# Danderson123/Amira

Measured on AMD Instinct MI355X. Metric: gene-mers/s to corrected GeneMerGraph, higher is better.
Workload: dtype int32; 1 GPU; synthetic 1M reads x 60 genes, k=5, 20k-gene vocab: build + error-correction sweep (build, filter(3,1), correct, build, clip(5), correct, build); reads_per_gpu=1000000, genes_per_read=60, k=5, vocab=20000, gene_mers_per_gpu=56000000, final_nodes=472478, final_edges=1054844, multi_gpu=n/a

## Files before the change

amira_amd/csrc/amg_correct.h:

```cpp
#pragma once
#include "amg_device.h"

enum { RC_SKIP = 0, RC_COPY = 1, RC_DROP = 2, RC_TRIM = 3, RC_GAPPED = 4, RC_KEEP_ORIG = 5 };

struct CorrArgs {
  const int* tokens;
  const long long* read_off;
  const int* tok_node;
  const signed char* tok_dir;
  const unsigned char* read_fix;
  const long long* p0s;
  const long long* p0e;
  const long long* p1s;
  const long long* p1e;
  long long n0;
  const long long* pos_off;
  const long long* read_len;
  long long n_reads;
  int k, flip, have_pos;
  unsigned int* gflag;
  unsigned long long* max_bound;
  unsigned long long* lmask;
  unsigned long long* n_runs;
  unsigned char* cls;
  unsigned char* cls_final;
  int* r_start;
  int* r_end;
  unsigned int* bound;
  const long long* tmp_off;
  unsigned int* new_len;
  int* tmp_tok;
};

__device__ __forceinline__ void pos_base(const CorrArgs& a, long long off, const long long*& gs, const long long*& ge) {
  if (off < a.n0) {
    gs = a.p0s + off;
    ge = a.p0e + off;
  } else {
    gs = a.p1s + (off - a.n0);
    ge = a.p1e + (off - a.n0);
  }
}

__device__ __forceinline__ long long bcast_i64(long long v, int lane) {
  const unsigned int lo = (unsigned int)__builtin_amdgcn_readlane((int)(unsigned int)v, lane);
  const unsigned int hi = (unsigned int)__builtin_amdgcn_readlane((int)(unsigned int)((unsigned long long)v >> 32), lane);
  return (long long)(((unsigned long long)hi << 32) | lo);
}

__device__ __forceinline__ void wave_sync() {
  __builtin_amdgcn_fence(__ATOMIC_ACQ_REL, "wavefront");
  __builtin_amdgcn_wave_barrier();
}

struct __attribute__((aligned(16))) GapRec {
  int r, L0, start, end;
  long long t0, dst;
  unsigned long long mask;
  long long pad;
};

__device__ __forceinline__ unsigned long long gap_run_ends(unsigned long long lv, int start, int end) {
  const unsigned long long inside =
      (end >= 63 ? ~0ull : ((1ull << (end + 1)) - 1ull)) & ~((1ull << (start & 63)) - 1ull);
  return ~lv & inside & (lv >> 1);
}
__device__ __forceinline__ void gap_run_terminals(unsigned long long lv, int i, int& ps, int& pe) {
  ps = 63 - __clzll((long long)(lv & ((1ull << i) - 1ull)));
  pe = i + 1;
}

struct GapArgs {
  CorrArgs a;
  GView g;
  const GapRec* rec;
  const int* gapped_reads;
  long long n_gapped;
  int* pool;
  unsigned long long pool_cap;
  unsigned long long* pool_used;
  unsigned long long* status;
  int* cand;
  unsigned int cand_stride;
  unsigned char* final_cls;
  unsigned char* need_slow;
  const int* gq;
  const int4* qres;
  const int* qpool;
};

#define GF_MAXW 128
#define GF_MAXGAP 16
#define GF_POOL 384
#define GF_CAND 136
#define GF_MAXCOMBO 256
#define GM_INLINE 64
#define LEAN_CHUNK 32
#define CLS_READS 64
#define PACK_READS 64
enum {
  GS_NOT_TRIED = 1,
  GS_WINDOWS = 2,
  GS_RUNS = 3,
  GS_MEMO_UNFIT = 4,
  GS_RECORDS = 5,
  GS_COMBOS = 6,
  GS_CAND = 7,
  GS_CODES = 8
};
enum {
  GL_NO_SLOTS = 1,
  GL_ANSWERS = 2,
  GL_LONG = 3,
  GL_OTHER = 4,
  GL_CODES = 5
};

#define NWF_MAX_M 64
#define NWF_MAX_N 128
__device__ __forceinline__ bool nw_fast_ok(long long N, long long M) {
  return N <= NWF_MAX_N && M <= NWF_MAX_M && N > 0 && M > 0;
}

struct __attribute__((aligned(16))) NwRec {
  int r, M, N, pad;
  long long t0, dst;
  long long pdst;
  long long poff;
};

struct NwArgs {
  CorrArgs a;
  const NwRec* rec;
  long long* o_gs;
  long long* o_ge;
  const int* gapped_reads;
  long long n_gapped;
  const unsigned char* final_cls;
  const long long* big_off;
  unsigned char* big_buf;
  int allow_fast;
  int shortcuts;
  unsigned char* route;
};
enum { NW_ROUTE_NONE = 0, NW_ROUTE_EQUAL = 1, NW_ROUTE_CERT = 2, NW_ROUTE_FILL = 3, NW_ROUTE_LDS = 4, NW_ROUTE_GLOBAL = 5 };

struct PackArgs {
  CorrArgs a;
  const long long* new_idx;
  const long long* new_off;
  const unsigned char* final_cls;
  int* o_tok;
  long long* o_off;
  int* o_orig;
  unsigned char* o_changed;
  long long* o_src;
  const long long* pos_new;
  long long* o_posoff;
  long long* o_rl;
  long long out_reads, out_tokens;
  unsigned long long* dead_kept;
};

struct CorrSwitches {
  bool gap_memo;
  bool fast_gapped;
  bool lean_gapped;
  int fast_nw;
  int nw_shortcuts;
  const char* node_bound;
  bool routes;
  const char* gap_pool;
  const char* memo_spill;
};

struct CorrScratch {
  size_t per_read = 0;
  unsigned char *cls = nullptr, *final_cls = nullptr;
  int *r_start = nullptr, *r_end = nullptr;
  long long *nw_size = nullptr, *nw_off = nullptr;
  unsigned int *bound = nullptr, *new_len = nullptr, *flag = nullptr;
  long long *tmp_off = nullptr, *new_idx = nullptr, *new_off = nullptr;
  int* tmp_tok = nullptr;
  long long *plen = nullptr, *poffs = nullptr, *pos_new = nullptr;
  unsigned long long *max_bound = nullptr, *n_general = nullptr;
  unsigned long long* n_runs = nullptr;
  unsigned long long* dead_kept = nullptr;
  bool count_alive = false;
  DevBuf* glist = nullptr;
  DevBuf* cand = nullptr;
  DevBuf* pool = nullptr;
  DevBuf* need_slow = nullptr;
};

struct CorrCounts {
  long long tmp_total = 0, n_gapped = 0, total_runs = 0;
  unsigned long long max_bound = 0;
  bool carry = false;
  long long out_reads = 0, out_tokens = 0, big_total = 0, pos_total = 0;
  unsigned long long n_general = 0;
  long long n_queries = 0;
  int pool_retries = 0;
  bool lean_ran = false, fast_ran = false, memo = false;
};

static void fill_pos_args(amg_ctx* c, CorrArgs& a) {
  a.p0s = c->have_pos ? c->gene_start.as<long long>() : nullptr;
  a.p0e = c->have_pos ? c->gene_end.as<long long>() : nullptr;
  a.p1s = c->pos1_s.as<long long>();
  a.p1e = c->pos1_e.as<long long>();
  a.n0 = c->pos_n0;
  a.pos_off = (c->have_pos && !c->pos_identity) ? c->pos_off.as<long long>() : nullptr;
}

void corr_classify_launch(amg_ctx* c, const CorrArgs& a);
int corr_gapped(amg_ctx* c, const CorrSwitches& sw, const CorrScratch& S, const CorrArgs& a, CorrCounts& n);
int corr_nw_sizes(amg_ctx* c, const CorrSwitches& sw, const CorrScratch& S, const CorrArgs& a, long long n_gapped,
                  FetchList& shape);
int corr_grow_pos_pools(amg_ctx* c, const CorrCounts& n);
int corr_positions(amg_ctx* c, const CorrSwitches& sw, const CorrScratch& S, const CorrArgs& a, const CorrCounts& n,
                   unsigned char* route = nullptr);

int routes_begin(amg_ctx* c);
int routes_gapped(amg_ctx* c, const CorrScratch& S, const CorrCounts& n, const unsigned char* need_slow, const int* gq);
int routes_nw(amg_ctx* c, const CorrScratch& S, const CorrCounts& n);
int routes_end(amg_ctx* c, const CorrCounts& n);
```

amira_amd/csrc/amg_correct.hip:

```cpp
#include "amg_correct.h"

__global__ __launch_bounds__(256) void k_count_alive(const unsigned char* __restrict__ alive, long long n,
                                                     unsigned long long* out) {
  __shared__ unsigned int s_part[4];
  unsigned int c = 0;
  for (long long i = ((long long)blockIdx.x * blockDim.x + threadIdx.x) * 4; i < n; i += (long long)gridDim.x * blockDim.x * 4) {
    if (i + 4 <= n) {
      const unsigned int w = *reinterpret_cast<const unsigned int*>(alive + i);
      c += __popc(w & 0x01010101u);
    } else {
      for (long long j = i; j < n; ++j) c += alive[j] ? 1u : 0u;
    }
  }
  for (int d = 32; d > 0; d >>= 1) c += (unsigned int)__shfl_xor((int)c, d, 64);
  if ((threadIdx.x & 63) == 0) s_part[threadIdx.x >> 6] = c;
  __syncthreads();
  if (threadIdx.x == 0 && (s_part[0] | s_part[1] | s_part[2] | s_part[3]))
    atomicAdd(out, (unsigned long long)s_part[0] + s_part[1] + s_part[2] + s_part[3]);
}

__global__ __launch_bounds__(256) void k_corr_pack(PackArgs A) {
  const CorrArgs& a = A.a;
  const int lane = threadIdx.x & 63;
  const long long r = ((long long)blockIdx.x * 4 + (threadIdx.x >> 6)) * PACK_READS + lane;
  if (blockIdx.x == 0 && threadIdx.x == 0) A.o_off[A.out_reads] = A.out_tokens;
  long long dst = 0, src = 0;
  int n = 0;
  unsigned int dead = 0;
  if (r < a.n_reads && a.new_len[r] > 0) {
    dst = A.new_off[r];
    n = (int)a.new_len[r];
    const unsigned char fc = A.final_cls[r];
    if (fc == RC_KEEP_ORIG) {
      const long long nw = a.read_off[r + 1] - a.read_off[r] - a.k + 1;
      dead = nw <= 64 ? (unsigned int)(nw - __popcll(a.lmask[r])) : (unsigned int)nw;
    }
    long long poff = 0;
    if (fc == RC_GAPPED) {
      src = a.tmp_off[r] | (1ll << 62);
      if (a.have_pos) poff = A.pos_new[r];
    } else {
      const long long cut = fc == RC_TRIM ? a.r_start[r] : 0;
      src = a.read_off[r] + cut;
      if (a.have_pos) poff = (a.pos_off ? a.pos_off[r] : a.read_off[r]) + cut;
    }
    const long long q = A.new_idx[r];
    A.o_off[q] = dst;
    A.o_orig[q] = (int)r;
    A.o_changed[q] = (fc == RC_TRIM || fc == RC_GAPPED) ? 1 : 0;
    A.o_src[q] = fc == RC_GAPPED ? -1ll : src;
    if (a.have_pos) A.o_posoff[q] = poff;
    if (a.read_len) A.o_rl[q] = a.read_len[r];
  }
  if (__ballot(dead != 0u) != 0ull) {
    for (int d = 32; d > 0; d >>= 1) dead += (unsigned int)__shfl_xor((int)dead, d, 64);
    if (lane == 0) atomicAdd(A.dead_kept + 16 * (blockIdx.x & 15), (unsigned long long)dead);
  }
  if (__ballot(n > 0) == 0ull) return;
  for (int j0 = 0; j0 < PACK_READS; j0 += 4) {
    const int* sp[4];
    long long d[4];
    int nn[4], vt[4];
#pragma unroll
    for (int j = 0; j < 4; ++j) {
      nn[j] = __builtin_amdgcn_readlane(n, j0 + j);
      const long long sj = bcast_i64(src, j0 + j);
      d[j] = bcast_i64(dst, j0 + j);
      sp[j] = ((sj >> 62) & 1 ? a.tmp_tok : a.tokens) + (sj & ~(1ll << 62));
    }
#pragma unroll
    for (int j = 0; j < 4; ++j)
      if (lane < nn[j]) vt[j] = sp[j][lane];
#pragma unroll
    for (int j = 0; j < 4; ++j)
      if (lane < nn[j]) A.o_tok[d[j] + lane] = vt[j];
#pragma unroll
    for (int j = 0; j < 4; ++j)
      for (int i = 64 + lane; i < nn[j]; i += 64)
        A.o_tok[d[j] + i] = sp[j][i];
  }
}

static CorrSwitches read_switches() {
  auto is_one = [](const char* name) {
    const char* v = getenv(name);
    return v && v[0] == '1';
  };
  CorrSwitches sw;
  sw.gap_memo = !is_one("AMG_NO_GAP_MEMO");
  sw.fast_gapped = !is_one("AMG_NO_FAST_GAPPED");
  sw.lean_gapped = !is_one("AMG_NO_LEAN_GAPPED");
  sw.fast_nw = !is_one("AMG_NO_FAST_NW");
  sw.nw_shortcuts = !is_one("AMG_NW_NO_SHORTCUT");
  sw.node_bound = getenv("AMG_TEST_NODE_BOUND");
  sw.routes = is_one("AMG_CORR_ROUTES");
  sw.gap_pool = getenv("AMG_TEST_GAP_POOL");
  sw.memo_spill = getenv("AMG_TEST_MEMO_SPILL");
  return sw;
}

static int plan_per_read(amg_ctx* c, CorrScratch& S) {
  const size_t per_read = (size_t)(c->n_reads + 2);
  AMGCHK(c->s0.ensure(per_read * (1 + 1) + 64));
  AMGCHK(c->s1.ensure(per_read * sizeof(int) * 2 + per_read * sizeof(long long) * 2 + 64));
  AMGCHK(c->s2.ensure(per_read * sizeof(unsigned int) * 3));
  AMGCHK(c->s3.ensure(per_read * sizeof(long long) * 3));
  AMGCHK(c->gm_mask.ensure(per_read * sizeof(unsigned long long)));
  AMGCHK(c->gm_ctr.ensure((16 + 256 + 256 + 16) * sizeof(unsigned long long)));
  S.per_read = per_read;
  S.cls = c->s0.as<unsigned char>();
  S.final_cls = S.cls + per_read;
  S.r_start = c->s1.as<int>();
  S.r_end = S.r_start + per_read;
  S.nw_size = reinterpret_cast<long long*>(((uintptr_t)(S.r_end + per_read) + 15) & ~(uintptr_t)15);
  S.nw_off = S.nw_size + per_read;
  S.bound = c->s2.as<unsigned int>();
  S.new_len = S.bound + per_read;
  S.flag = S.new_len + per_read;
  S.tmp_off = c->s3.as<long long>();
  S.new_idx = S.tmp_off + per_read;
  S.new_off = S.new_idx + per_read;
  S.max_bound = S.n_general = c->status.as<unsigned long long>() + ST_MISC;
  S.n_runs = c->gm_ctr.as<unsigned long long>() + 16;
  S.dead_kept = S.n_runs + 256;
  S.count_alive = c->n_nodes >= (1ll << 20);
  S.glist = &c->c_orig;
  S.cand = &c->c_gstart;
  S.pool = &c->c_gend;
  S.need_slow = &c->c_changed;
  return AMG_OK;
}

static int plan_staging(amg_ctx* c, CorrScratch& S, long long tmp_total) {
  AMGCHK(c->c_tokens_buf.ensure((size_t)(tmp_total + 4) * sizeof(int)));
  AMGCHK(c->s4.ensure((size_t)(tmp_total + 4) * sizeof(int)));
  S.tmp_tok = c->s4.as<int>();
  return AMG_OK;
}

static int plan_positions(amg_ctx* c, CorrScratch& S, long long n_gapped) {
  AMGCHK(c->s5.ensure((size_t)(2 * (n_gapped + 2) + c->n_reads + 2) * sizeof(long long)));
  S.plen = c->s5.as<long long>();
  S.poffs = S.plen + (n_gapped + 2);
  S.pos_new = S.poffs + (n_gapped + 2);
  return AMG_OK;
}

static void corr_args(amg_ctx* c, const CorrScratch& S, CorrArgs& a) {
  a.tokens = c->tokens.as<int>();
  a.read_off = c->read_off.as<long long>();
  a.tok_node = c->tok_node.as<int>();
  a.tok_dir = c->tok_dir.as<signed char>();
  a.read_fix = c->read_fix.as<unsigned char>();
  fill_pos_args(c, a);
  a.read_len = c->have_read_len ? c->read_len.as<long long>() : nullptr;
  a.n_reads = c->n_reads;
  a.k = c->k;
  a.flip = c->two_v - 1;
  a.have_pos = c->have_pos ? 1 : 0;
  a.gflag = S.flag;
  a.max_bound = S.max_bound;
  a.lmask = c->gm_mask.as<unsigned long long>();
  a.n_runs = S.n_runs;
  a.cls = S.cls;
  a.cls_final = S.final_cls;
  a.r_start = S.r_start;
  a.r_end = S.r_end;
  a.bound = S.bound;
  a.tmp_off = S.tmp_off;
  a.new_len = S.new_len;
  a.tmp_tok = S.tmp_tok;
}

static int corr_classify(amg_ctx* c, const CorrScratch& S, const CorrArgs& a, CorrCounts& n) {
  hipStream_t st = c->stream;
  const long long R = c->n_reads;
  {
    ClearList cl;
    cl.add(S.bound, S.per_read * sizeof(unsigned int) * 3);
    cl.add(S.max_bound, sizeof(unsigned long long));
    cl.add(S.n_runs, (256 + 256 + 16) * sizeof(unsigned long long));
    AMGCHK(clear_many(c, cl));
  }
  if (R > 0) corr_classify_launch(c, a);
  if (S.count_alive)
    hipLaunchKernelGGL(k_count_alive, dim3(128), dim3(256), 0, st, c->node_alive.as<unsigned char>(), c->n_nodes,
                       S.dead_kept + 256);
  AMGCHK(prim_exscan_u32_pair(c, S.bound, S.tmp_off, S.flag, S.new_idx, (size_t)R));
  FetchList l;
  l.add(S.tmp_off + R);
  l.add(S.max_bound);
  l.add(S.new_idx + R);
  for (int i = 0; i < 16; ++i) l.add(S.n_runs + 16 * i);
  unsigned long long v[3 + 16];
  AMGCHK(fetch(c, l, v));
  n.tmp_total = (long long)v[0];
  n.max_bound = v[1];
  n.n_gapped = (long long)v[2];
  for (int i = 0; i < 16; ++i) n.total_runs += (long long)v[3 + i];
  n.carry = n.n_gapped > 0 && c->have_pos;
  return AMG_OK;
}

static int corr_shape(amg_ctx* c, const CorrSwitches& sw, CorrScratch& S, const CorrArgs& a, CorrCounts& n) {
  const long long R = c->n_reads;
  AMGCHK(prim_exscan_keep_and_len(c, S.new_len, S.new_idx, S.new_off, (size_t)R));
  FetchList shape;
  shape.add(S.new_idx + R);
  shape.add(S.new_off + R);
  if (n.carry) {
    AMGCHK(plan_positions(c, S, n.n_gapped));
    AMGCHK(corr_nw_sizes(c, sw, S, a, n.n_gapped, shape));
  }
  unsigned long long v[5] = {0, 0, 0, 0, 0};
  AMGCHK(fetch(c, shape, v));
  n.out_reads = (long long)v[0];
  n.out_tokens = (long long)v[1];
  n.big_total = (long long)v[2];
  n.pos_total = (long long)v[3];
  n.n_general = v[4];
  return AMG_OK;
}

static int ensure_outputs(amg_ctx* c, const CorrCounts& n) {
  AMGCHK(c->c_tokens_buf.ensure((size_t)(n.out_tokens + 64) * sizeof(int)));
  AMGCHK(c->c_read_off.ensure((size_t)(n.out_reads + 2) * sizeof(long long)));
  AMGCHK(c->c_orig.ensure((size_t)(n.out_reads + 2) * sizeof(int)));
  AMGCHK(c->c_changed.ensure((size_t)(n.out_reads + 2)));
  AMGCHK(c->c_src.ensure((size_t)(n.out_reads + 2) * sizeof(long long)));
  if (c->have_pos) AMGCHK(c->c_pos_off.ensure((size_t)(n.out_reads + 2) * sizeof(long long)));
  if (c->have_read_len) AMGCHK(c->c_read_len.ensure((size_t)(n.out_reads + 2) * sizeof(long long)));
  return AMG_OK;
}

static int corr_pack(amg_ctx* c, const CorrScratch& S, const CorrArgs& a, const CorrCounts& n) {
  PackArgs Pk;
  Pk.a = a;
  Pk.new_idx = S.new_idx;
  Pk.new_off = S.new_off;
  Pk.final_cls = S.final_cls;
  Pk.o_tok = c->c_tokens_buf.as<int>();
  Pk.o_off = c->c_read_off.as<long long>();
// ... 90 lines not shown
```

amira_amd/csrc/amg_correct_gapped.hip:

```cpp
#include "amg_correct.h"
#include "amg_wave_dfs.h"

__global__ __launch_bounds__(256) void k_corr_classify(CorrArgs a) {
  const long long rbase = ((long long)blockIdx.x * 4 + (threadIdx.x >> 6)) * CLS_READS;
  if (rbase >= a.n_reads) return;
  const int lane = threadIdx.x & 63;
  const long long r = rbase + lane;
  const bool have = r < a.n_reads;
  const long long t0 = have ? a.read_off[r] : 0;
  const long long n = have ? (a.read_off[r + 1] - t0) - a.k + 1 : 0;
  const bool look = have && n > 0 && a.read_fix[r] != 0;
  unsigned long long lv = 0;
  unsigned long long todo = __ballot(look && n <= 64);
  while (todo) {
    int who[4];
    long long tj[4];
    int nj[4], v[4];
#pragma unroll
    for (int q = 0; q < 4; ++q) {
      who[q] = todo ? __ffsll((long long)todo) - 1 : -1;
      if (todo) todo &= todo - 1ull;
      tj[q] = who[q] >= 0 ? bcast_i64(t0, who[q]) : 0;
      nj[q] = who[q] >= 0 ? __builtin_amdgcn_readlane((int)n, who[q]) : 0;
    }
#pragma unroll
    for (int q = 0; q < 4; ++q) v[q] = lane < nj[q] ? a.tok_node[tj[q] + lane] : -1;
#pragma unroll
    for (int q = 0; q < 4; ++q) {
      const unsigned long long m = __ballot(v[q] >= 0);
      if (lane == who[q]) lv = m;
    }
  }
  long long first = n, last = -1;
  unsigned int runs = 0, live = 0;
  if (look && n <= 64) {
    first = lv ? (long long)__ffsll((long long)lv) - 1 : n;
    last = lv ? 63 - (long long)__clzll((long long)lv) : -1;
    live = (unsigned int)__popcll(lv);
    const unsigned long long inside =
        lv ? ((last == 63 ? ~0ull : ((1ull << (last + 1)) - 1ull)) & ~((1ull << first) - 1ull)) : 0ull;
    runs = (unsigned int)__popcll(~lv & inside & (lv >> 1));
  }
  unsigned long long big = __ballot(look && n > 64);
  while (big) {
    const int w = __ffsll((long long)big) - 1;
    big &= big - 1ull;
    const long long tw = bcast_i64(t0, w), nw = bcast_i64(n, w);
    long long f = nw, l = -1;
    for (long long i = lane; i < nw; i += 64)
      if (a.tok_node[tw + i] >= 0) {
        f = f < i ? f : i;
        l = l > i ? l : i;
      }
    for (int d = 32; d > 0; d >>= 1) {
      const long long f2 = __shfl_xor(f, d, 64), l2 = __shfl_xor(l, d, 64);
      f = f < f2 ? f : f2;
      l = l > l2 ? l : l2;
    }
    unsigned int ru = 0, li = 0;
    if (l >= 0) {
      for (long long i = f + lane; i <= l; i += 64) {
        const bool none = a.tok_node[tw + i] < 0;
        li += none ? 0u : 1u;
        if (none && a.tok_node[tw + i + 1] >= 0) ++ru;
      }
      for (int d = 32; d > 0; d >>= 1) {
        ru += __shfl_xor(ru, d, 64);
        li += __shfl_xor(li, d, 64);
      }
    }
    if (lane == w) {
      first = f;
      last = l;
      runs = ru;
      live = li;
    }
  }
  const long long L = n + a.k - 1;
  unsigned char cls;
  int start = 0, end = -1;
  unsigned int bound = 0;
  unsigned int len_out = 0;
  if (n <= 0) {
    cls = RC_SKIP;
  } else if (!look) {
    cls = RC_COPY;
    len_out = (unsigned int)L;
  } else if (last < 0) {
    cls = RC_DROP;
  } else {
    start = (int)first;
    end = (int)last;
    if (runs == 0) {
      cls = RC_TRIM;
      len_out = (unsigned int)(end - start + a.k);
    } else {
      cls = RC_GAPPED;
      const unsigned int b1 = live + runs * (unsigned int)(2 * a.k) + (unsigned int)a.k;
      bound = b1 > (unsigned int)L ? b1 : (unsigned int)L;
    }
  }
  if (have) {
    a.cls[r] = cls;
    a.cls_final[r] = cls;
    a.r_start[r] = start;
    a.r_end[r] = end;
    a.bound[r] = bound;
    a.new_len[r] = len_out;
    a.gflag[r] = cls == RC_GAPPED ? 1u : 0u;
    a.lmask[r] = (cls == RC_GAPPED && n <= 64) ? lv : 0ull;
  }
  unsigned int mb = (have && cls == RC_GAPPED) ? bound : 0u;
  unsigned int nr = (have && cls == RC_GAPPED) ? runs : 0u;
  for (int d = 32; d > 0; d >>= 1) {
    const unsigned int o = (unsigned int)__shfl_xor((int)mb, d, 64);
    mb = mb > o ? mb : o;
    nr += (unsigned int)__shfl_xor((int)nr, d, 64);
  }
  if (lane == 0 && (unsigned long long)mb > *a.max_bound) atomicMax(a.max_bound, (unsigned long long)mb);
  if (lane == 0 && nr) atomicAdd(a.n_runs + 16 * (blockIdx.x & 15), (unsigned long long)nr);
}

void corr_classify_launch(amg_ctx* c, const CorrArgs& a) {
  hipLaunchKernelGGL(k_corr_classify, dim3(nblk(a.n_reads, 4 * CLS_READS)), dim3(256), 0, c->stream, a);
}

#define DFS_MAX (2 * AMG_MAX_K + 4)

struct PathSink {
  int* buf;
  long long used;
  int n_paths;
};

__device__ void dfs_paths(const GView& g, int s, int sdir, int e, int distance, PathSink* sink) {
  int node[DFS_MAX], dir[DFS_MAX];
  long long cur[DFS_MAX], lim[DFS_MAX];
  int depth = 0;
  node[0] = s;
  dir[0] = sdir;
  bool entering = true;
  while (depth >= 0) {
    if (entering) {
      int L = depth + 1;
      if (node[depth] == e && L <= distance) {
        if (sink->buf) {
          int* o = sink->buf + sink->used;
          o[0] = L;
          for (int j = 0; j < L; ++j) {
            o[1 + j] = node[j];
            o[1 + L + j] = dir[j];
          }
        }
        sink->used += 1 + 2 * L;
        sink->n_paths += 1;
        --depth;
        entering = false;
        continue;
      }
      if (L - 1 > distance) {
        --depth;
        entering = false;
        continue;
      }
      long long row = 2ll * node[depth] + (dir[depth] == 1 ? 0 : 1);
      const int4 rw = g.lrows[row];
      cur[depth] = rw.x;
      lim[depth] = rw.x + rw.y;
      entering = false;
    }
    bool pushed = false;
    while (cur[depth] < lim[depth]) {
      const int2 ent = g.lent[cur[depth]++];
      int t = ent.x;
      bool seen = false;
      for (int j = 0; j <= depth; ++j) seen = seen || (node[j] == t);
      if (seen) continue;
      node[depth + 1] = t;
      dir[depth + 1] = ent.y;
      ++depth;
      entering = true;
      pushed = true;
      break;
    }
    if (!pushed) --depth;
  }
}

__device__ __forceinline__ int oriented_tok(const GView& g, int n, int d, int j) {
  const int* nt = g.n_tok + (long long)n * g.k;
  return d == 1 ? nt[j] : g.flip - nt[g.k - 1 - j];
}

struct GapIter {
  long long t0;
  const int* tok_node;
  int start, end, i;
  int ps, pe;
  __device__ bool next() {
    while (i <= end) {
      int idx = i++;
      if (tok_node[t0 + idx] < 0) {
        if (tok_node[t0 + idx - 1] >= 0) ps = idx - 1;
        if (tok_node[t0 + idx + 1] >= 0) {
          pe = idx + 1;
          return true;
        }
      }
    }
    return false;
  }
};

__device__ __forceinline__ bool cand_better(int shared, unsigned long long csum, int n, int best_shared,
                                            unsigned long long best_sum, unsigned long long best_len) {
  return shared > best_shared || (shared == best_shared && csum * best_len > best_sum * (unsigned long long)n);
}

__device__ int build_candidate(const GapArgs& A, long long t0, int start, int end, const int* rec,
                               int n_gaps, unsigned long long combo, int* out_node, signed char* out_dir) {
  int n = 0;
  int q = 0;
  int i = start;
  int prev_pe = -1;
  while (i <= end) {
    if (q < n_gaps && rec[4 * q] == i) {
      int ps = rec[4 * q], pe = rec[4 * q + 1], np = rec[4 * q + 2];
      unsigned long long div = 1;
      for (int j = q + 1; j < n_gaps; ++j) div *= (unsigned long long)rec[4 * j + 2];
      int pick = (int)((combo / div) % (unsigned long long)np);
      const int* p = A.pool + rec[4 * q + 3];
      for (int s = 0; s < pick; ++s) p += 1 + 2 * p[0];
      int L = p[0];
      if (prev_pe == ps && n > 0) --n;
      for (int j = 0; j < L; ++j) {
        out_node[n] = p[1 + j];
        out_dir[n] = (signed char)p[1 + L + j];
        ++n;
      }
      prev_pe = pe;
      i = pe;
      ++q;
      if (!(q < n_gaps && rec[4 * q] == pe)) i = pe + 1;
    } else {
      out_node[n] = A.a.tok_node[t0 + i];
      out_dir[n] = A.a.tok_dir[t0 + i];
      ++n;
      ++i;
    }
  }
  return n;
}

__global__ __launch_bounds__(64) void k_corr_gapped(GapArgs A) {
  const CorrArgs& a = A.a;
  const GView& g = A.g;
  const long long gtid = (long long)blockIdx.x * blockDim.x + threadIdx.x;
  const long long gstride = (long long)gridDim.x * blockDim.x;
  int* my = A.cand + gtid * (long long)A.cand_stride;
  for (long long gi = gtid; gi < A.n_gapped; gi += gstride) {
    if (!A.need_slow[gi]) continue;
    const long long r = A.gapped_reads[gi];
    const long long t0 = a.read_off[r];
    const int L0 = (int)(a.read_off[r + 1] - t0);
    const int start = a.r_start[r], end = a.r_end[r];
    const long long dst = a.tmp_off[r];
    int n_gaps = 0;
    long long need = 0;
    bool dead_end = false;
    {
      GapIter it{t0, a.tok_node, start, end, start, -1, -1};
      while (it.next()) {
        PathSink sink{nullptr, 0, 0};
        dfs_paths(g, a.tok_node[t0 + it.ps], a.tok_dir[t0 + it.ps], a.tok_node[t0 + it.pe], 2 * g.k, &sink);
        if (sink.n_paths == 0) dead_end = true;
        need += sink.used;
        ++n_gaps;
      }
    }
    bool keep_orig = dead_end;
    int* rec = nullptr;
    if (!keep_orig) {
      unsigned long long want = (unsigned long long)need + 4ull * n_gaps;
      unsigned long long base = atomicAdd(A.pool_used, want);
      if (base + want > A.pool_cap) {
        A.status[ST_OVERFLOW] = 3;
        a.new_len[r] = 0;
        continue;
      }
      rec = A.pool + base;
      int* wr = rec + 4 * n_gaps;
      GapIter it{t0, a.tok_node, start, end, start, -1, -1};
      int q = 0;
      while (it.next()) {
        PathSink sink{wr, 0, 0};
        dfs_paths(g, a.tok_node[t0 + it.ps], a.tok_dir[t0 + it.ps], a.tok_node[t0 + it.pe], 2 * g.k, &sink);
        rec[4 * q] = it.ps;
        rec[4 * q + 1] = it.pe;
        rec[4 * q + 2] = sink.n_paths;
        rec[4 * q + 3] = (int)(wr - A.pool);
        wr += sink.used;
        ++q;
      }
    }
    if (keep_orig) {
      a.new_len[r] = (unsigned int)L0;
      A.final_cls[r] = RC_KEEP_ORIG;
      continue;
    }
    unsigned long long n_combo = 1;
    for (int q = 0; q < n_gaps; ++q) {
      n_combo *= (unsigned long long)rec[4 * q + 2];
      if (n_combo > (1ull << 40)) n_combo = 1ull << 40;
    }
    const int cap_nodes = (int)a.bound[r];
    int* c_node = my;
    signed char* c_dir = reinterpret_cast<signed char*>(my + cap_nodes);
    int* c_gene = my + cap_nodes + (cap_nodes + 3) / 4;
    int best_shared = 0;
    unsigned long long best_sum = 0, best_len = 1;
    int best_n = -1;
    for (unsigned long long combo = 0; combo < n_combo; ++combo) {
      int n = build_candidate(A, t0, start, end, rec, n_gaps, combo, c_node, c_dir);
      int ng = 0;
      for (int j = 0; j < g.k - 1; ++j) c_gene[ng++] = oriented_tok(g, c_node[0], c_dir[0], j);
      unsigned long long csum = 0;
      for (int j = 0; j < n; ++j) {
        c_gene[ng++] = oriented_tok(g, c_node[j], c_dir[j], g.k - 1);
        csum += g.n_cov[c_node[j]];
      }
      int shared = 0;
      for (int j = 0; j < ng; ++j) {
        int tk = c_gene[j];
        bool dup = false;
        for (int q = 0; q < j && !dup; ++q) dup = (c_gene[q] == tk);
        if (dup) continue;
        bool hit = false;
        for (int q = 0; q < L0 && !hit; ++q) hit = (a.tokens[t0 + q] == tk);
        shared += hit ? 1 : 0;
      }
      if (cand_better(shared, csum, n, best_shared, best_sum, best_len)) {
        best_shared = shared;
        best_sum = csum;
        best_len = (unsigned long long)n;
        best_n = ng;
        for (int j = 0; j < ng; ++j) a.tmp_tok[dst + j] = c_gene[j];
      }
    }
    a.new_len[r] = (unsigned int)best_n;
  }
}


struct GapVisit {
  int e, distance, run, lane;
  int *pool, *used;
  int n_paths;
  bool overflow;
  __device__ __forceinline__ int enter(int, int L, int cur_node, int, int my_node, int my_dir) {
    if (cur_node == e && L <= distance) {
      const int off = *used;
      if (off + 2 + 2 * L <= GF_POOL) {
        if (lane == 0) {
          pool[off] = run;
          pool[off + 1] = L;
        }
        if (lane < L) {
          pool[off + 2 + lane] = my_node;
          pool[off + 2 + L + lane] = my_dir;
        }
      } else {
        overflow = true;
      }
      wave_sync();
      if (lane == 0) *used = off + 2 + 2 * L;
      wave_sync();
      ++n_paths;
      return WD_RETREAT;
    }
    return L - 1 > distance ? WD_RETREAT : WD_EXPAND;
  }
};

__device__ __forceinline__ int dfs_paths_wave(const GView& g, int s, int sdir, int e, int distance, int run, int* pool,
                                              int* used, int lane) {
  GapVisit v{e, distance, run, lane, pool, used, 0, false};
  wave_dfs(g, s, sdir, lane, v);
  return v.overflow ? -1 : v.n_paths;
}

__device__ __forceinline__ unsigned long long gap_query_key(int s, int sdir, int e) {
  return (1ull << 63) | ((unsigned long long)(unsigned int)s << 32) | ((unsigned long long)(unsigned int)e << 1) |
         (sdir == 1 ? 1ull : 0ull);
}

__global__ __launch_bounds__(256) void k_gap_queries(const GapRec* __restrict__ rec, long long n_gapped, int k,
                                                      const int* __restrict__ tok_node,
                                                      const signed char* __restrict__ tok_dir,
                                                      unsigned long long* qtab, unsigned int qmask,
                                                      unsigned long long* ctr ,
                                                      int* __restrict__ qlist, int* __restrict__ gq,
                                                      unsigned long long* status) {
  __shared__ int s_list[256 * GF_MAXGAP];
  __shared__ unsigned int s_n;
  __shared__ unsigned long long s_base;
  if (threadIdx.x == 0) s_n = 0;
  __syncthreads();
  const long long gi = (long long)blockIdx.x * blockDim.x + threadIdx.x;
  if (gi < n_gapped) {
    const GapRec q = rec[gi];
    int* my = gq + gi * GF_MAXGAP;
    const int nwin = q.L0 - k + 1;
    const unsigned long long lv = q.mask;
    unsigned long long ends = gap_run_ends(lv, q.start, q.end);
    if (nwin > 64 || lv == 0ull || __popcll(ends) > GF_MAXGAP) {
      my[0] = -1;
    } else {
      int j = 0;
      while (ends) {
        int ps, pe;
        gap_run_terminals(lv, __ffsll((long long)ends) - 1, ps, pe);
        ends &= ends - 1ull;
        const unsigned long long key = gap_query_key(tok_node[q.t0 + ps], (int)tok_dir[q.t0 + ps], tok_node[q.t0 + pe]);
        unsigned int idx = (unsigned int)mix64(key) & qmask;
        int slot = -1;
        for (unsigned int probes = 0; probes <= qmask; ++probes) {
          unsigned long long cur = qtab[idx];
          if (cur == 0ull) {
            cur = atomicCAS(qtab + idx, 0ull, key);
            if (cur == 0ull) {
              s_list[atomicAdd(&s_n, 1u)] = (int)idx;
              cur = key;
            }
          }
          if (cur == key) {
            slot = (int)idx;
            break;
          }
          idx = (idx + 1) & qmask;
        }
        if (slot < 0) status[ST_OVERFLOW] = 7;
        my[j++] = slot;
      }
    }
  }
  __syncthreads();
  const unsigned int n = s_n;
  if (n == 0) return;
  if (threadIdx.x == 0) s_base = atomicAdd(ctr, (unsigned long long)n);
  __syncthreads();
  for (unsigned int i = threadIdx.x; i < n; i += 256) qlist[s_base + i] = s_list[i];
}

__global__ __launch_bounds__(64, 8) void k_gap_dfs(GView g, const int* __restrict__ qlist, long long n_queries,
                                                    const unsigned long long* __restrict__ qtab,
                                                    unsigned long long* pool_used, unsigned long long pool_cap,
                                                    int* __restrict__ qpool, int4* __restrict__ qres,
                                                    int* __restrict__ qgene) {
  __shared__ int s_pool[GF_POOL];
  __shared__ int s_used;
  const long long qi = blockIdx.x;
  if (qi >= n_queries) return;
  const int lane = threadIdx.x;
  const int slot = qlist[qi];
  const unsigned long long key = qtab[slot];
  const int s = (int)((key >> 32) & 0x7fffffffull), e = (int)((key >> 1) & 0x7fffffffull);
  const int sdir = (key & 1ull) ? 1 : -1;
  if (lane == 0) s_used = 0;
  wave_sync();
  const int np = dfs_paths_wave(g, s, sdir, e, 2 * g.k, 0, s_pool, &s_used, lane);
  wave_sync();
  const int used = s_used;
  int4 res = make_int4(0, -1, 0, 0);
  if (np >= 0) {
    unsigned long long off = (unsigned long long)qi * GM_INLINE;
    if (used > GM_INLINE) {
      if (lane == 0) off = (unsigned long long)n_queries * GM_INLINE + atomicAdd(pool_used, (unsigned long long)used);
      off = (unsigned long long)bcast_i64((long long)off, 0);
    }
    if (off + (unsigned long long)used <= pool_cap) {
      for (int i = lane; i < used; i += 64) qpool[off + i] = s_pool[i];
      res = make_int4((int)off, used, np, 0);
      if (np == 1 && used <= GM_INLINE) {
        const int len = s_pool[1];
        if (lane < len) qgene[off + 2 + lane] = oriented_tok(g, s_pool[2 + lane], s_pool[2 + len + lane], g.k - 1);
      }
    }
  }
  if (lane == 0) qres[slot] = res;
}

#define GL_GROUP 16
#define GL_THREADS 256
__device__ __forceinline__ int row_scan_incl(int v) {
  v += __builtin_amdgcn_update_dpp(0, v, 0x111, 0xf, 0xf, false);
  v += __builtin_amdgcn_update_dpp(0, v, 0x112, 0xf, 0xf, false);
  v += __builtin_amdgcn_update_dpp(0, v, 0x114, 0xf, 0xf, false);
  v += __builtin_amdgcn_update_dpp(0, v, 0x118, 0xf, 0xf, false);
  return v;
}

__global__ __launch_bounds__(GL_THREADS) void k_corr_gapped_lean(GapArgs A, const int* __restrict__ qgene,
                                                                  unsigned char* __restrict__ left) {
  __shared__ int4 s_run[GL_THREADS / GL_GROUP][GL_GROUP];
  __shared__ int s_tk[GL_THREADS / GL_GROUP][64 + AMG_MAX_K];
  const CorrArgs& a = A.a;
  const int k = A.g.k;
  const int lane = threadIdx.x & 63, l16 = threadIdx.x & (GL_GROUP - 1), grp = threadIdx.x / GL_GROUP;
  const int sh = lane & ~(GL_GROUP - 1);
  const long long gi = (long long)blockIdx.x * (GL_THREADS / GL_GROUP) + grp;
  const bool have = gi < A.n_gapped;
  GapRec rec;
  rec.r = 0; rec.L0 = 0; rec.start = 0; rec.end = -1; rec.t0 = 0; rec.dst = 0; rec.mask = 0ull; rec.pad = 0;
  int slot = have ? A.gq[gi * GF_MAXGAP + l16] : -1;
  if (have) rec = A.rec[gi];
  const unsigned long long lv = rec.mask;
  const int nwin = rec.L0 - k + 1;
  bool ok = have && nwin <= 64 && lv != 0ull;
  const int first = rec.start, last = rec.end;
  unsigned long long ends = ok ? gap_run_ends(lv, first, last) : 0ull;
  const int n_gaps = __popcll(ends);
  ok = ok && n_gaps >= 1 && n_gaps <= GF_MAXGAP;
  const bool mine = ok && l16 < n_gaps;
  if (!mine) slot = -1;
  int4 res = make_int4(0, -1, 0, 0);
  if (mine && slot >= 0) res = A.qres[slot];
  if (ok) {
    const int span = last + k - first;
    for (int i = l16; i < span; i += GL_GROUP) s_tk[grp][i] = a.tokens[rec.t0 + first + i];
  }
  int ps = 0, pe = 0;
  if (mine) {
    unsigned long long e = ends;
    for (int j = 0; j < l16; ++j) e &= e - 1ull;
    gap_run_terminals(lv, __ffsll((long long)e) - 1, ps, pe);
  }
  const int len = (mine && res.y >= 4) ? (res.y - 2) >> 1 : 0;
  const bool good = !mine || (slot >= 0 && res.z == 1 && res.y >= 6 && res.y <= GM_INLINE && len >= 2);
  const unsigned int bad16 = (unsigned int)((__ballot(!good) >> sh) & 0xffffull);
  const bool multi = !good && slot >= 0 && res.z != 1;
  const bool toolong = !good && slot >= 0 && res.z == 1 && res.y > GM_INLINE;
  const unsigned int multi16 = (unsigned int)((__ballot(multi) >> sh) & 0xffffull);
  const unsigned int long16 = (unsigned int)((__ballot(toolong) >> sh) & 0xffffull);
  const int why = !ok ? GL_NO_SLOTS : multi16 ? GL_ANSWERS : long16 ? GL_LONG : GL_OTHER;
  ok = ok && bad16 == 0u;
  const int ps_next = __builtin_amdgcn_update_dpp(-1, ps, 0x101, 0xf, 0xf, false);
  const int shared = (mine && l16 + 1 < n_gaps && ps_next == pe) ? 1 : 0;
// ... 175 lines not shown
  for (int q = lane; q < ng; q += 64) {
    const int idx = q < g.k - 1 ? 0 : q - (g.k - 1);
    const int j = q < g.k - 1 ? q : g.k - 1;
    S.gene[q] = oriented_tok(g, S.cnode[idx], S.cdir[idx], j);
  }
  if (rank) {
    for (int q = lane; q < n; q += 64) csum += g.n_cov[S.cnode[q]];
    for (int d = 32; d > 0; d >>= 1) csum += __shfl_xor(csum, d, 64);
  }
  wave_sync();
  if (rank) {
    for (int q = lane; q < ng; q += 64) {
      const int tk = S.gene[q];
      bool dup = false;
      for (int w = 0; w < q && !dup; ++w) dup = (S.gene[w] == tk);
      bool hit = false;
      if (!dup)
        for (int w = 0; w < L0 && !hit; ++w) hit = (S.tok[w] == tk);
      shared += hit ? 1 : 0;
    }
    for (int d = 32; d > 0; d >>= 1) shared += __shfl_xor(shared, d, 64);
  }
}

__device__ __forceinline__ void gf_hand_down(const GapArgs& A, long long gi, int lane, int why) {
  if (lane == 0) A.need_slow[gi] = (unsigned char)why;
}

__device__ __forceinline__ void gapped_fast_read(const GapArgs& A, long long gi, int lane, GfLds& S) {
  const CorrArgs& a = A.a;
  const GView& g = A.g;
  const GapRec rec = A.rec[gi];
  const int nwin = rec.L0 - g.k + 1;
  if (nwin > GF_MAXW) return gf_hand_down(A, gi, lane, GS_WINDOWS);
  const int myslot = (A.gq && lane < GF_MAXGAP) ? A.gq[gi * GF_MAXGAP + lane] : -1;
  gf_stage(a, rec, nwin, lane, S);
  const int n_gaps = gf_list_runs(rec.start, rec.end, lane, S);
  if (n_gaps > GF_MAXGAP) return gf_hand_down(A, gi, lane, GS_RUNS);
  wave_sync();
  const int unfit = __builtin_amdgcn_readfirstlane(myslot) >= 0 ? gf_paths_from_memo(A, myslot, n_gaps, lane, S)
                                                                : gf_paths_by_search(g, n_gaps, lane, S);
  if (unfit) return gf_hand_down(A, gi, lane, unfit);
  wave_sync();
  bool dead_end;
  const unsigned long long n_combo = gf_count_combos(S, n_gaps, dead_end);
  if (dead_end) {
    if (lane == 0) {
      a.new_len[rec.r] = (unsigned int)rec.L0;
      A.final_cls[rec.r] = RC_KEEP_ORIG;
    }
    return;
  }
  if (n_combo > GF_MAXCOMBO) return gf_hand_down(A, gi, lane, GS_COMBOS);
  const int used = S.used;
  int best_shared = 0, best_ng = -1;
  unsigned long long best_sum = 0, best_len = 1;
  for (unsigned long long combo = 0; combo < n_combo; ++combo) {
    const int n = gf_build_candidate(S, rec.start, rec.end, n_gaps, used, combo, lane);
    wave_sync();
    if (n < 0) return gf_hand_down(A, gi, lane, GS_CAND);
    int shared;
    unsigned long long csum;
    gf_spell_and_score(g, S, n, rec.L0, n_combo > 1, lane, shared, csum);
    if (n_combo == 1 || cand_better(shared, csum, n, best_shared, best_sum, best_len)) {
      best_shared = shared;
      best_sum = csum;
      best_len = (unsigned long long)n;
      best_ng = n + g.k - 1;
      for (int q = lane; q < best_ng; q += 64) S.best[q] = S.gene[q];
    }
    wave_sync();
  }
  for (int q = lane; q < best_ng; q += 64) a.tmp_tok[rec.dst + q] = S.best[q];
  if (lane == 0) a.new_len[rec.r] = (unsigned int)best_ng;
}

__global__ __launch_bounds__(64 * GF_WPB, 8) void k_corr_gapped_fast(GapArgs A, const unsigned char* __restrict__ left) {
  __shared__ GfLds s_lds;
  const int lane = (int)threadIdx.x;
  if (!left) {
    if ((long long)blockIdx.x < A.n_gapped) gapped_fast_read(A, (long long)blockIdx.x, lane, s_lds);
    return;
  }
  const long long base = (long long)blockIdx.x * LEAN_CHUNK;
  const bool mine = lane < LEAN_CHUNK && base + lane < A.n_gapped && left[base + lane] != 0;
  unsigned long long todo = __ballot(mine);
  while (todo) {
    const int b = __ffsll((long long)todo) - 1;
    todo &= todo - 1ull;
    gapped_fast_read(A, base + b, lane, s_lds);
    wave_sync();
  }
}

__global__ void k_scatter_gapped(const unsigned int* __restrict__ flag, const long long* __restrict__ pos,
                                 long long n_reads, int* __restrict__ out, const long long* __restrict__ read_off,
                                 const int* __restrict__ r_start, const int* __restrict__ r_end,
                                 const long long* __restrict__ tmp_off, const unsigned long long* __restrict__ lmask,
                                 GapRec* __restrict__ rec) {
  long long r = (long long)blockIdx.x * blockDim.x + threadIdx.x;
  if (r >= n_reads || !flag[r]) return;
  const long long gi = pos[r];
  out[gi] = (int)r;
  GapRec q;
  q.r = (int)r;
  q.t0 = read_off[r];
  const long long len = read_off[r + 1] - q.t0;
  q.L0 = (int)(len > 0x7fffffff ? 0x7fffffff : len);
  q.start = r_start[r];
  q.end = r_end[r];
  q.dst = tmp_off[r];
  q.mask = lmask[r];
  q.pad = 0;
  rec[gi] = q;
}

static int gap_memo(amg_ctx* c, const CorrSwitches& sw, const CorrArgs& a, CorrCounts& n, const int** gq) {
  hipStream_t st = c->stream;
  const long long n_gapped = n.n_gapped, total_runs = n.total_runs;
  *gq = nullptr;
  const uint64_t qslots = pow2_at_least((uint64_t)total_runs * 2 + 16);
  AMGCHK(c->gm_tab.ensure((size_t)qslots * sizeof(unsigned long long)));
  AMGCHK(c->gm_res.ensure((size_t)qslots * sizeof(int4)));
  AMGCHK(c->gm_list.ensure((size_t)(total_runs + 1) * sizeof(int)));
  AMGCHK(c->gm_q.ensure((size_t)(n_gapped + 1) * GF_MAXGAP * sizeof(int)));
  {
    ClearList cl;
    cl.add(c->gm_tab.p, (size_t)qslots * sizeof(unsigned long long));
    cl.add(c->gm_ctr.p, 16 * sizeof(unsigned long long));
    cl.add(c->status.as<unsigned long long>() + ST_OVERFLOW, sizeof(unsigned long long));
    AMGCHK(clear_many(c, cl));
  }
  hipLaunchKernelGGL(k_gap_queries, dim3(nblk(n_gapped, 256)), dim3(256), 0, st, c->gap_rec.as<GapRec>(), n_gapped,
                     c->k, a.tok_node, a.tok_dir, c->gm_tab.as<unsigned long long>(), (unsigned int)(qslots - 1),
                     c->gm_ctr.as<unsigned long long>(), c->gm_list.as<int>(), c->gm_q.as<int>(),
                     c->status.as<unsigned long long>());
  unsigned long long v[2] = {0, 0};
  {
    FetchList l;
    l.add(c->gm_ctr.p);
    l.add(c->status.as<unsigned long long>() + ST_OVERFLOW);
    AMGCHK(fetch(c, l, v));
  }
  if (v[1]) return amg_fail(AMG_E_HIP, "correct_reads: path memo table full");
  const long long n_queries = (long long)v[0];
  unsigned long long qcap = (unsigned long long)n_queries * (GM_INLINE + 32ull) + 4096ull;
  if (sw.memo_spill) {
    const unsigned long long lo = (unsigned long long)n_queries * GM_INLINE + strtoull(sw.memo_spill, nullptr, 10);
    qcap = lo < qcap ? lo : qcap;
  }
  if (qcap > 0x7fffffffull) return AMG_OK;
  AMGCHK(c->gm_pool.ensure((size_t)qcap * sizeof(int)));
  AMGCHK(c->gm_gene.ensure((size_t)qcap * sizeof(int)));
  if (n_queries > 0)
    hipLaunchKernelGGL(k_gap_dfs, dim3((unsigned int)n_queries), dim3(64), 0, st, make_view(c), c->gm_list.as<int>(),
                       n_queries, c->gm_tab.as<unsigned long long>(), c->gm_ctr.as<unsigned long long>() + 1, qcap,
                       c->gm_pool.as<int>(), c->gm_res.as<int4>(), c->gm_gene.as<int>());
  *gq = c->gm_q.as<int>();
  n.n_queries = n_queries;
  return AMG_OK;
}

int corr_gapped(amg_ctx* c, const CorrSwitches& sw, const CorrScratch& S, const CorrArgs& a, CorrCounts& n) {
  hipStream_t st = c->stream;
  const long long R = c->n_reads, n_gapped = n.n_gapped;
  AMGCHK(S.glist->ensure((size_t)(n_gapped + 1) * sizeof(int)));
  AMGCHK(c->gap_rec.ensure((size_t)(n_gapped + 1) * sizeof(GapRec)));
  hipLaunchKernelGGL(k_scatter_gapped, dim3(nblk(R, 256)), dim3(256), 0, st, S.flag, S.new_idx, R,
                     S.glist->as<int>(), a.read_off, S.r_start, S.r_end, S.tmp_off, a.lmask, c->gap_rec.as<GapRec>());
  const int* gq = nullptr;
  if (n.total_runs > 0 && sw.gap_memo) AMGCHK(gap_memo(c, sw, a, n, &gq));
  const unsigned int threads_total = 64u * 2048u;
  unsigned int cand_stride = (unsigned int)(2 * n.max_bound + (n.max_bound + 3) / 4 + c->k + 16);
  AMGCHK(S.cand->ensure((size_t)threads_total * cand_stride * sizeof(int)));
  unsigned long long pool_cap = 1ull << 22;
  if (sw.gap_pool) {
    const unsigned long long lo = strtoull(sw.gap_pool, nullptr, 10);
    pool_cap = lo < pool_cap ? lo : pool_cap;
  }
  AMGCHK(S.need_slow->ensure((size_t)n_gapped + 64));
  unsigned char* need_slow = S.need_slow->as<unsigned char>();
  for (int attempt = 0;; ++attempt) {
    AMGCHK(S.pool->ensure((size_t)pool_cap * sizeof(int)));
    unsigned long long* used = c->status.as<unsigned long long>() + ST_COMPACT_A;
    ClearList gcl;
    gcl.add(c->status.p, ST_WORDS * sizeof(unsigned long long));
    GapArgs G;
    G.a = a;
    G.g = make_view(c);
    G.rec = c->gap_rec.as<GapRec>();
    G.gapped_reads = S.glist->as<int>();
    G.n_gapped = n_gapped;
    G.pool = S.pool->as<int>();
    G.pool_cap = pool_cap;
    G.pool_used = used;
    G.status = c->status.as<unsigned long long>();
    G.cand = S.cand->as<int>();
    G.cand_stride = cand_stride;
    G.final_cls = S.final_cls;
    G.need_slow = need_slow;
    G.gq = gq;
    G.qres = c->gm_res.as<int4>();
    G.qpool = c->gm_pool.as<int>();
    if (attempt == 0) {
      gcl.add(need_slow, ((size_t)n_gapped + 4) & ~(size_t)3, sw.fast_gapped ? 0u : 0x01010101u);
      AMGCHK(clear_many(c, gcl));
      if (sw.fast_gapped && gq && sw.lean_gapped) {
        n.lean_ran = true;
        AMGCHK(c->gm_fail.ensure((size_t)n_gapped + 64));
        hipLaunchKernelGGL(k_corr_gapped_lean, dim3(nblk(n_gapped, GL_THREADS / GL_GROUP)), dim3(GL_THREADS), 0, st, G,
                           c->gm_gene.as<int>(), c->gm_fail.as<unsigned char>());
        hipLaunchKernelGGL(k_corr_gapped_fast, dim3(nblk(n_gapped, LEAN_CHUNK)), dim3(64 * GF_WPB), 0, st, G,
                           c->gm_fail.as<unsigned char>());
      } else if (sw.fast_gapped) {
        hipLaunchKernelGGL(k_corr_gapped_fast, dim3((unsigned int)n_gapped), dim3(64 * GF_WPB), 0, st, G,
                           (const unsigned char*)nullptr);
      }
    } else {
      AMGCHK(clear_many(c, gcl));
    }
    unsigned int blocks = (unsigned int)((n_gapped + 63) / 64);
    if (blocks > 2048u) blocks = 2048u;
    hipLaunchKernelGGL(k_corr_gapped, dim3(blocks), dim3(64), 0, st, G);
    unsigned long long hs[ST_WORDS];
    AMGCHK(fetch_status(c, hs));
    if (!hs[ST_OVERFLOW]) break;
    if (attempt >= 8) return amg_fail(AMG_E_OVERFLOW, "correct_reads: path pool overflow");
    pool_cap = hs[ST_COMPACT_A] * 2 + (1ull << 20);
    n.pool_retries = attempt + 1;
  }
  if (sw.routes) AMGCHK(routes_gapped(c, S, n, need_slow, gq));
  return AMG_OK;
}
```

Measured before the change: 10.39 billion gene-mers/s.

## Run gap-path DFS one query per lane with wave fallback for overflows

```diff
diff --git a/amira_amd/csrc/amg_correct.h b/amira_amd/csrc/amg_correct.h
--- a/amira_amd/csrc/amg_correct.h
+++ b/amira_amd/csrc/amg_correct.h
@@ -164,6 +164,7 @@
 
 struct CorrSwitches {
   bool gap_memo;
+  bool gap_dfs_wave;
   bool fast_gapped;
   bool lean_gapped;
   int fast_nw;
@@ -221,6 +222,11 @@
 int corr_positions(amg_ctx* c, const CorrSwitches& sw, const CorrScratch& S, const CorrArgs& a, const CorrCounts& n,
                    unsigned char* route = nullptr);
 
+bool gap_dfs_lanes_fits(int k);
+void gap_dfs_lanes_launch(amg_ctx* c, const int* qlist, long long n_queries, const unsigned long long* qtab,
+                          unsigned long long* pool_used, unsigned long long pool_cap, int* qpool, int4* qres,
+                          int* qgene);
+
 int routes_begin(amg_ctx* c);
 int routes_gapped(amg_ctx* c, const CorrScratch& S, const CorrCounts& n, const unsigned char* need_slow, const int* gq);
 int routes_nw(amg_ctx* c, const CorrScratch& S, const CorrCounts& n);
diff --git a/amira_amd/csrc/amg_correct.hip b/amira_amd/csrc/amg_correct.hip
--- a/amira_amd/csrc/amg_correct.hip
+++ b/amira_amd/csrc/amg_correct.hip
@@ -88,6 +88,7 @@
   };
   CorrSwitches sw;
   sw.gap_memo = !is_one("AMG_NO_GAP_MEMO");
+  sw.gap_dfs_wave = is_one("AMG_GAP_DFS_WAVE");
   sw.fast_gapped = !is_one("AMG_NO_FAST_GAPPED");
   sw.lean_gapped = !is_one("AMG_NO_LEAN_GAPPED");
   sw.fast_nw = !is_one("AMG_NO_FAST_NW");
diff --git a/amira_amd/csrc/amg_correct_gapped.hip b/amira_amd/csrc/amg_correct_gapped.hip
--- a/amira_amd/csrc/amg_correct_gapped.hip
+++ b/amira_amd/csrc/amg_correct_gapped.hip
@@ -1,5 +1,5 @@
 #include "amg_correct.h"
-#include "amg_wave_dfs.h"
+#include "amg_gap_search.h"
 
 __global__ __launch_bounds__(256) void k_corr_classify(CorrArgs a) {
   const long long rbase = ((long long)blockIdx.x * 4 + (threadIdx.x >> 6)) * CLS_READS;
@@ -187,11 +187,6 @@
   }
 }
 
-__device__ __forceinline__ int oriented_tok(const GView& g, int n, int d, int j) {
-  const int* nt = g.n_tok + (long long)n * g.k;
-  return d == 1 ? nt[j] : g.flip - nt[g.k - 1 - j];
-}
-
 struct GapIter {
   long long t0;
   const int* tok_node;
@@ -351,48 +346,6 @@
   }
 }
 
-
-struct GapVisit {
-  int e, distance, run, lane;
-  int *pool, *used;
-  int n_paths;
-  bool overflow;
-  __device__ __forceinline__ int enter(int, int L, int cur_node, int, int my_node, int my_dir) {
-    if (cur_node == e && L <= distance) {
-      const int off = *used;
-      if (off + 2 + 2 * L <= GF_POOL) {
-        if (lane == 0) {
-          pool[off] = run;
-          pool[off + 1] = L;
-        }
-        if (lane < L) {
-          pool[off + 2 + lane] = my_node;
-          pool[off + 2 + L + lane] = my_dir;
-        }
-      } else {
-        overflow = true;
-      }
-      wave_sync();
-      if (lane == 0) *used = off + 2 + 2 * L;
-      wave_sync();
-      ++n_paths;
-      return WD_RETREAT;
-    }
-    return L - 1 > distance ? WD_RETREAT : WD_EXPAND;
-  }
-};
-
-__device__ __forceinline__ int dfs_paths_wave(const GView& g, int s, int sdir, int e, int distance, int run, int* pool,
-                                              int* used, int lane) {
-  GapVisit v{e, distance, run, lane, pool, used, 0, false};
-  wave_dfs(g, s, sdir, lane, v);
-  return v.overflow ? -1 : v.n_paths;
-}
-
-__device__ __forceinline__ unsigned long long gap_query_key(int s, int sdir, int e) {
-  return (1ull << 63) | ((unsigned long long)(unsigned int)s << 32) | ((unsigned long long)(unsigned int)e << 1) |
-         (sdir == 1 ? 1ull : 0ull);
-}
 
 __global__ __launch_bounds__(256) void k_gap_queries(const GapRec* __restrict__ rec, long long n_gapped, int k,
                                                       const int* __restrict__ tok_node,
@@ -874,7 +827,11 @@
   if (qcap > 0x7fffffffull) return AMG_OK;
   AMGCHK(c->gm_pool.ensure((size_t)qcap * sizeof(int)));
   AMGCHK(c->gm_gene.ensure((size_t)qcap * sizeof(int)));
-  if (n_queries > 0)
+  if (n_queries > 0 && !sw.gap_dfs_wave && gap_dfs_lanes_fits(c->k))
+    gap_dfs_lanes_launch(c, c->gm_list.as<int>(), n_queries, c->gm_tab.as<unsigned long long>(),
+                         c->gm_ctr.as<unsigned long long>() + 1, qcap, c->gm_pool.as<int>(), c->gm_res.as<int4>(),
+                         c->gm_gene.as<int>());
+  else if (n_queries > 0)
     hipLaunchKernelGGL(k_gap_dfs, dim3((unsigned int)n_queries), dim3(64), 0, st, make_view(c), c->gm_list.as<int>(),
                        n_queries, c->gm_tab.as<unsigned long long>(), c->gm_ctr.as<unsigned long long>() + 1, qcap,
                        c->gm_pool.as<int>(), c->gm_res.as<int4>(), c->gm_gene.as<int>());
diff --git a/amira_amd/csrc/amg_gap_memo.hip b/amira_amd/csrc/amg_gap_memo.hip
--- /dev/null
+++ b/amira_amd/csrc/amg_gap_memo.hip
@@ -0,0 +1,155 @@
+#include "amg_gap_search.h"
+
+#define GDL_THREADS 256
+#define GDL_DEPTH 16
+#define GDL_STEPS 4096
+#define GDL_DIR_BIT 0x80000000u
+
+__global__ __launch_bounds__(GDL_THREADS) void k_gap_dfs_lanes(GView g, const int* __restrict__ qlist, long long n_queries,
+                                                                const unsigned long long* __restrict__ qtab,
+                                                                unsigned long long* pool_used, unsigned long long pool_cap,
+                                                                int* __restrict__ qpool, int4* __restrict__ qres,
+                                                                int* __restrict__ qgene) {
+  __shared__ unsigned int s_node[GDL_DEPTH][GDL_THREADS];
+  __shared__ int s_cur[GDL_DEPTH][GDL_THREADS];
+  __shared__ int s_lim[GDL_DEPTH][GDL_THREADS];
+  __shared__ int s_pool[GDL_THREADS / 64][GF_POOL];
+  __shared__ int s_used[GDL_THREADS / 64];
+  const int t = threadIdx.x, lane = t & 63, w = t >> 6;
+  const long long qi = (long long)blockIdx.x * GDL_THREADS + t;
+  if (qi - lane >= n_queries) return;
+  const bool have = qi < n_queries;
+  const int distance = 2 * g.k;
+  int slot = 0, s = 0, sdir = 1, e = 0;
+  if (have) {
+    slot = qlist[qi];
+    const unsigned long long key = qtab[slot];
+    s = (int)((key >> 32) & 0x7fffffffull);
+    e = (int)((key >> 1) & 0x7fffffffull);
+    sdir = (key & 1ull) ? 1 : -1;
+  }
+  const long long off = qi * GM_INLINE;
+  bool flagged = have && (unsigned long long)(off + GM_INLINE) > pool_cap;
+  int used = 0, n_paths = 0;
+  if (have && !flagged) {
+    int depth = 0, cur = 0, lim = 0;
+    int2 first_ent = make_int2(-1, 0);
+    bool entering = true;
+    s_node[0][t] = (unsigned int)s | (sdir == 1 ? GDL_DIR_BIT : 0u);
+    int step = 0;
+    for (; step < GDL_STEPS && depth >= 0; ++step) {
+      if (entering) {
+        entering = false;
+        const unsigned int nw = s_node[depth][t];
+        const int node = (int)(nw & ~GDL_DIR_BIT);
+        const int L = depth + 1;
+        if (node == e && L <= distance) {
+          if (used + 2 + 2 * L > GM_INLINE) {
+            flagged = true;
+            break;
+          }
+          int* o = qpool + off + used;
+          unsigned int pw[GDL_DEPTH];
+          int gene[GDL_DEPTH];
+#pragma unroll
+          for (int j = 0; j < GDL_DEPTH; ++j) {
+            pw[j] = j < L ? s_node[j][t] : 0u;
+            gene[j] = 0;
+            if (j < L && n_paths == 0)
+              gene[j] = oriented_tok(g, (int)(pw[j] & ~GDL_DIR_BIT), (pw[j] & GDL_DIR_BIT) ? 1 : -1, g.k - 1);
+          }
+          o[0] = 0;
+          o[1] = L;
+#pragma unroll
+          for (int j = 0; j < GDL_DEPTH; ++j)
+            if (j < L) {
+              o[2 + j] = (int)(pw[j] & ~GDL_DIR_BIT);
+              o[2 + L + j] = (pw[j] & GDL_DIR_BIT) ? 1 : -1;
+              if (n_paths == 0) qgene[off + 2 + j] = gene[j];
+            }
+          used += 2 + 2 * L;
+          ++n_paths;
+        } else if (L - 1 <= distance) {
+          const int4 rw = g.lrows[2ll * node + ((nw & GDL_DIR_BIT) ? 0 : 1)];
+          cur = rw.x;
+          lim = rw.x + rw.y;
+          first_ent = make_int2(rw.z, rw.w);
+          continue;
+        }
+        --depth;
+        if (depth >= 0) {
+          cur = s_cur[depth][t];
+          lim = s_lim[depth][t];
+        }
+        first_ent.x = -1;
+      } else if (cur < lim) {
+        int2 ent = first_ent;
+        if (first_ent.x < 0) ent = g.lent[cur];
+        first_ent.x = -1;
+        ++cur;
+        bool seen = false;
+#pragma unroll
+        for (int j = 0; j < GDL_DEPTH; ++j) seen = seen || (j <= depth && (int)(s_node[j][t] & ~GDL_DIR_BIT) == ent.x);
+        if (seen) continue;
+        if (depth + 1 >= GDL_DEPTH) {
+          flagged = true;
+          break;
+        }
+        s_cur[depth][t] = cur;
+        s_lim[depth][t] = lim;
+        ++depth;
+        s_node[depth][t] = (unsigned int)ent.x | (ent.y == 1 ? GDL_DIR_BIT : 0u);
+        entering = true;
+      } else {
+        --depth;
+        if (depth >= 0) {
+          cur = s_cur[depth][t];
+          lim = s_lim[depth][t];
+        }
+        first_ent.x = -1;
+      }
+    }
+    if (depth >= 0) flagged = true;
+    if (!flagged) qres[slot] = make_int4((int)off, used, n_paths, 0);
+  }
+  unsigned long long todo = __ballot(flagged);
+  for (int turn = 0; turn < 64 && todo; ++turn) {
+    const int b = __ffsll((long long)todo) - 1;
+    todo &= todo - 1ull;
+    const int bs = __builtin_amdgcn_readlane(s, b), be = __builtin_amdgcn_readlane(e, b);
+    const int bdir = __builtin_amdgcn_readlane(sdir, b), bslot = __builtin_amdgcn_readlane(slot, b);
+    const long long bqi = qi - lane + b;
+    if (lane == 0) s_used[w] = 0;
+    wave_sync();
+    const int np = dfs_paths_wave(g, bs, bdir, be, distance, 0, s_pool[w], &s_used[w], lane);
+    wave_sync();
+    const int bused = s_used[w];
+    int4 res = make_int4(0, -1, 0, 0);
+    if (np >= 0) {
+      unsigned long long boff = (unsigned long long)bqi * GM_INLINE;
+      if (bused > GM_INLINE) {
+        if (lane == 0) boff = (unsigned long long)n_queries * GM_INLINE + atomicAdd(pool_used, (unsigned long long)bused);
+        boff = (unsigned long long)bcast_i64((long long)boff, 0);
+      }
+      if (boff + (unsigned long long)bused <= pool_cap) {
+        for (int i = lane; i < bused; i += 64) qpool[boff + i] = s_pool[w][i];
+        res = make_int4((int)boff, bused, np, 0);
+        if (np == 1 && bused <= GM_INLINE) {
+          const int len = s_pool[w][1];
+          if (lane < len) qgene[boff + 2 + lane] = oriented_tok(g, s_pool[w][2 + lane], s_pool[w][2 + len + lane], g.k - 1);
+        }
+      }
+    }
+    if (lane == 0) qres[bslot] = res;
+    wave_sync();
+  }
+}
+
+bool gap_dfs_lanes_fits(int k) { return 2 * k + 2 <= GDL_DEPTH; }
+
+void gap_dfs_lanes_launch(amg_ctx* c, const int* qlist, long long n_queries, const unsigned long long* qtab,
+                          unsigned long long* pool_used, unsigned long long pool_cap, int* qpool, int4* qres,
+                          int* qgene) {
+  hipLaunchKernelGGL(k_gap_dfs_lanes, dim3(nblk(n_queries, GDL_THREADS)), dim3(GDL_THREADS), 0, c->stream,
+                     make_view(c), qlist, n_queries, qtab, pool_used, pool_cap, qpool, qres, qgene);
+}
diff --git a/amira_amd/csrc/amg_gap_search.h b/amira_amd/csrc/amg_gap_search.h
--- /dev/null
+++ b/amira_amd/csrc/amg_gap_search.h
@@ -0,0 +1,50 @@
+#pragma once
+#include "amg_correct.h"
+#include "amg_wave_dfs.h"
+
+__device__ __forceinline__ int oriented_tok(const GView& g, int n, int d, int j) {
+  const int* nt = g.n_tok + (long long)n * g.k;
+  return d == 1 ? nt[j] : g.flip - nt[g.k - 1 - j];
+}
+
+struct GapVisit {
+  int e, distance, run, lane;
+  int *pool, *used;
+  int n_paths;
+  bool overflow;
+  __device__ __forceinline__ int enter(int, int L, int cur_node, int, int my_node, int my_dir) {
+    if (cur_node == e && L <= distance) {
+      const int off = *used;
+      if (off + 2 + 2 * L <= GF_POOL) {
+        if (lane == 0) {
+          pool[off] = run;
+          pool[off + 1] = L;
+        }
+        if (lane < L) {
+          pool[off + 2 + lane] = my_node;
+          pool[off + 2 + L + lane] = my_dir;
+        }
+      } else {
+        overflow = true;
+      }
+      wave_sync();
+      if (lane == 0) *used = off + 2 + 2 * L;
+      wave_sync();
+      ++n_paths;
+      return WD_RETREAT;
+    }
+    return L - 1 > distance ? WD_RETREAT : WD_EXPAND;
+  }
+};
+
+__device__ __forceinline__ int dfs_paths_wave(const GView& g, int s, int sdir, int e, int distance, int run, int* pool,
+                                              int* used, int lane) {
+  GapVisit v{e, distance, run, lane, pool, used, 0, false};
+  wave_dfs(g, s, sdir, lane, v);
+  return v.overflow ? -1 : v.n_paths;
+}
+
+__device__ __forceinline__ unsigned long long gap_query_key(int s, int sdir, int e) {
+  return (1ull << 63) | ((unsigned long long)(unsigned int)s << 32) | ((unsigned long long)(unsigned int)e << 1) |
+         (sdir == 1 ? 1ull : 0ull);
+}
```

Result: faster. 10.58 billion gene-mers/s (median of 6 runs) (+1.8%).
